# togheppi/pytorch-super-resolution-model-collection

Hardware: AMD Instinct MI355X
Metric: ESPCN x4 LR->HR images/sec (infer) (higher is better)
Workload: dtype f32 storage/accumulate; fp32-faithful products on the fp16 matrix cores: operands scaled by exact powers of two, split into two fp16 planes, 3 MFMAs per product (f16x3, ~3e-7 rms vs fp64, like fp32 MFMA); 1 GPU; c2: ESPCN x4 inference, 256x256 LR, batch 64 per GPU, fp32, random-init N(0,0.02); parallelism=replicas x1 (no collective)

## Files before the change

pytorch_super_resolution_model_collection_amd/csrc/conv_pair.hip:

```cpp
#include "srk_common.h"
#include "conv_problem.h"
#include "bf16_frag.h"
#include <type_traits>

namespace srk {

namespace {

constexpr int PR_TH = 8, PR_TW = 16, PR_HW = 18, PR_NPIX = 180, PR_NPIXP = 190;
constexpr int PR_XR = 14, PR_XC = 23, PR_XP = 24;
constexpr int PR_NSLOT = 3;
constexpr int PR_WL2 = 9 * 2 * 256;
constexpr int PR_HBUF = 8 * PR_NPIXP;
constexpr int PR_XBUF = 2 * PR_XR * PR_XP;
constexpr unsigned PR_SPIN_CAP = 1u << 18;
constexpr size_t PR_LDS = (size_t)PR_WL2 * 16 + (size_t)PR_NSLOT * PR_HBUF * 16 + (size_t)2 * PR_XBUF * 8 + 64;

__device__ unsigned g_pair_timeouts = 0;

typedef __attribute__((address_space(3))) unsigned pr_cnt_t;
typedef unsigned v4u_t __attribute__((ext_vector_type(4)));

struct PairParams {
  const float* x;
  const float* w1;
  const float* b1;
  const uint4* wq2;
  const float* w2_descale;
  const float* b2;
  float* y;
  const float* x_amax;
  float* y_amax;
  int N, H, W, OH, OW, tiles_x, img_tiles, ntiles;
  unsigned x_img_bytes, y_bytes;
};

__device__ __forceinline__ unsigned pr_peek(pr_cnt_t* p) {
  return (unsigned)__builtin_amdgcn_readfirstlane((int)__hip_atomic_load(p, __ATOMIC_RELAXED, __HIP_MEMORY_SCOPE_WORKGROUP));
}
__device__ __forceinline__ void pr_wait(pr_cnt_t* p, unsigned target, bool& dead) {
  if (!dead) {
    unsigned spins = 0;
    while ((int)(pr_peek(p) - target) < 0) {
      __builtin_amdgcn_s_sleep(1);
      if (++spins > PR_SPIN_CAP) {
        dead = true;
        break;
      }
    }
  }
  asm volatile("" ::: "memory");
}
__device__ __forceinline__ void pr_signal(pr_cnt_t* p) {
  asm volatile("" ::: "memory");
  if ((threadIdx.x & 63) == 0) __hip_atomic_fetch_add(p, 1u, __ATOMIC_RELAXED, __HIP_MEMORY_SCOPE_WORKGROUP);
  asm volatile("" ::: "memory");
}

__device__ __forceinline__ __amdgpu_buffer_rsrc_t pr_rsrc(const void* base, unsigned bytes) {
  const unsigned long long a = reinterpret_cast<unsigned long long>(base);
  const unsigned lo = __builtin_amdgcn_readfirstlane((unsigned)a), hi = __builtin_amdgcn_readfirstlane((unsigned)(a >> 32));
  void* p = reinterpret_cast<void*>(((unsigned long long)hi << 32) | lo);
  return __builtin_amdgcn_make_buffer_rsrc(p, (short)0, (int)__builtin_amdgcn_readfirstlane(bytes), 0x00020000);
}

__global__ __launch_bounds__(512, 1) void k_espcn_pair(PairParams B) {
  extern __shared__ __attribute__((aligned(16))) uint4 smem4[];
  uint4* wl2 = smem4;
  uint4* ring = smem4 + PR_WL2;
  uint2* xin_all = reinterpret_cast<uint2*>(ring + PR_NSLOT * PR_HBUF);
  pr_cnt_t* cnt = (pr_cnt_t*)(xin_all + 2 * PR_XBUF);
  const int tid = threadIdx.x, lane = tid & 63, wave = tid >> 6;
  const int grp = wave >> 2, gw = wave & 3, lt = tid & 255;
  const int j = lane & 15, kq = lane >> 4;
  uint2* xin = xin_all + grp * PR_XBUF;

  const float xmax = amax_read(B.x_amax);
  const int kx = amax_scale_exp(xmax);
  float wsum = 0.f, wmax = 0.f;
  {
    const float* wc = B.w1 + lane * 75;
    for (int i = 0; i < 75; ++i) {
      const float a = fabsf(wc[i]);
      wsum += a;
      wmax = fmaxf(wmax, a);
    }
  }
  const float bnd = wave_max(fabsf(B.b1[lane]) + wsum * xmax);
  const int kw1 = amax_scale_exp(wave_max(wmax));
  const int km = amax_scale_exp(bnd);
  const float sx1 = exp2i(kx), sw1 = exp2i(kw1), sxm = exp2i(km);
  const float dsc1 = exp2i(-kx) * exp2i(-kw1);
  const float dsc2 = exp2i(-km) * B.w2_descale[0];

  for (int e = tid; e < PR_WL2; e += 512) wl2[e] = B.wq2[e];
  if (tid < 8) cnt[tid] = 0u;

  const int nf1 = gw & 1, mh = gw >> 1;
  uint4 w1f[2][4][2];
#pragma unroll
  for (int cc = 0; cc < 2; ++cc) {
    const int co = cc * 32 + nf1 * 16 + j;
#pragma unroll
    for (int ks = 0; ks < 4; ++ks) {
      const int q = 4 * ks + kq, dy = q / 3, dx0 = 2 * (q - 3 * (q / 3));
      float f[8];
#pragma unroll
      for (int e = 0; e < 8; ++e) {
        const int dx = dx0 + (e >> 2), ci = e & 3;
        const bool on = q < 15 && ci < 3 && dx < 5;
        f[e] = on ? B.w1[((co * 3 + (on ? ci : 0)) * 5 + (on ? dy : 0)) * 5 + (on ? dx : 0)] : 0.f;
      }
      uint4 pl[2];
      split8h(f, sw1, pl);
      w1f[cc][ks][0] = pl[0];
      w1f[cc][ks][1] = pl[1];
    }
  }
  float b1v[2][4];
#pragma unroll
  for (int cc = 0; cc < 2; ++cc)
#pragma unroll
    for (int e = 0; e < 4; ++e) b1v[cc][e] = B.b1[cc * 32 + nf1 * 16 + 4 * kq + e];
  int koff[4], moff[6], mpix[6];
#pragma unroll
  for (int ks = 0; ks < 4; ++ks) {
    const int q = (4 * ks + kq) < 15 ? 4 * ks + kq : 14;
    koff[ks] = (q / 3) * PR_XP + 2 * (q - 3 * (q / 3));
  }
#pragma unroll
  for (int m = 0; m < 6; ++m) {
    const int p = (6 * mh + m) * 16 + j;
    mpix[m] = p;
    const int pc = p < PR_NPIX ? p : PR_NPIX - 1;
    moff[m] = (pc / PR_HW) * PR_XP + pc % PR_HW;
  }

  const int rh = gw >> 1, nf2 = gw & 1;
  const int pj = j < 4 ? 2 * j : (j < 12 ? 2 * j - 7 : 2 * j - 16);
  const int lane_b = (4 * rh) * PR_HW + pj + kq * PR_NPIXP;
  const int lane_a = kq * 32 + nf2 * 16 + j;
  float b2v[4];
#pragma unroll
  for (int e = 0; e < 4; ++e) b2v[e] = B.b2[nf2 * 16 + 4 * kq + e];

  const int nblk = gridDim.x, xcd = blockIdx.x & 7, bi = blockIdx.x >> 3;
  int first, count;
  {
    const int per_x = B.ntiles >> 3, rem_x = B.ntiles & 7;
    const int nb_x = (nblk + 7 - xcd) >> 3;
    const int tiles_x = per_x + (xcd < rem_x ? 1 : 0);
    const int start_x = xcd * per_x + (xcd < rem_x ? xcd : rem_x);
    first = start_x + bi;
    count = bi < tiles_x ? (tiles_x - bi + nb_x - 1) / nb_x : 0;
  }
  const int tstride = (nblk + 7 - xcd) >> 3;
  count = __builtin_amdgcn_readfirstlane(count);

  const __amdgpu_buffer_rsrc_t yr = pr_rsrc(B.y, B.y_bytes);
  const unsigned HW_ = (unsigned)(B.H * B.W);
  float xv[2][3];
  auto xload = [&](int i) {
    const bool valid = i < count;
    const int t = first + (valid ? i : 0) * tstride;
    const int n = t / B.img_tiles, rem = t - n * B.img_tiles;
    const int ty = rem / B.tiles_x, tx = rem - ty * B.tiles_x;
    const __amdgpu_buffer_rsrc_t xr = pr_rsrc(B.x + (size_t)n * 3 * HW_, B.x_img_bytes);
#pragma unroll
    for (int s = 0; s < 2; ++s) {
      const int q = lt + 256 * s, qy = q / PR_XC, qx = q - qy * PR_XC;
      const bool ok = valid && q < PR_XR * PR_XC;
      const unsigned o = ok ? 4u * (unsigned)((ty * PR_TH + qy) * B.W + tx * PR_TW + qx) : 0x80000000u;
#pragma unroll
      for (int c = 0; c < 3; ++c)
        xv[s][c] = __builtin_bit_cast(float, __builtin_amdgcn_raw_buffer_load_b32(xr, (int)(o + (ok ? 4u * c * HW_ : 0u)), 0, 0));
    }
  };
  bool dead = false;
  float amax = 0.f;
  xload(grp);
  __syncthreads();

  unsigned own = 0;
  for (int i = grp; i < count; i += 2, ++own) {
#pragma unroll
    for (int s = 0; s < 2; ++s) {
      const int q = lt + 256 * s;
      if (q < PR_XR * PR_XC) {
        const int qy = q / PR_XC, qx = q - qy * PR_XC;
        unsigned h01, m01, h2, m2;
        split2h(xv[s][0], xv[s][1], sx1, h01, m01);
        split2h(xv[s][2], 0.f, sx1, h2, m2);
        xin[qy * PR_XP + qx] = make_uint2(h01, h2);
        xin[PR_XR * PR_XP + qy * PR_XP + qx] = make_uint2(m01, m2);
      }
    }
    pr_signal(cnt + 6 + grp);
    xload(i + 2);
    pr_wait(cnt + 6 + grp, 4u * (own + 1), dead);

    f32x4 a1[2][6];
#pragma unroll
    for (int cc = 0; cc < 2; ++cc)
#pragma unroll
      for (int m = 0; m < 6; ++m) a1[cc][m] = (f32x4){0.f, 0.f, 0.f, 0.f};
#pragma unroll
    for (int ks = 0; ks < 4; ++ks) {
#pragma unroll
      for (int m = 0; m < 6; ++m) {
        const int pa = moff[m] + koff[ks];
        const uint2 h0 = xin[pa], h1 = xin[pa + 1];
        const uint2 l0 = xin[PR_XR * PR_XP + pa], l1 = xin[PR_XR * PR_XP + pa + 1];
        const uint4 xh = make_uint4(h0.x, h0.y, h1.x, h1.y), xm = make_uint4(l0.x, l0.y, l1.x, l1.y);
#pragma unroll
        for (int cc = 0; cc < 2; ++cc) {
          a1[cc][m] = mfma16h(w1f[cc][ks][0], xm, a1[cc][m]);
          a1[cc][m] = mfma16h(w1f[cc][ks][1], xh, a1[cc][m]);
          a1[cc][m] = mfma16h(w1f[cc][ks][0], xh, a1[cc][m]);
        }
      }
    }
#pragma unroll
    for (int cc = 0; cc < 2; ++cc) {
      const unsigned st = 2u * (unsigned)i + cc, slot = st % PR_NSLOT, use = st / PR_NSLOT;
      pr_wait(cnt + 3 + slot, 4u * use, dead);
      unsigned char* hb = reinterpret_cast<unsigned char*>(ring + slot * PR_HBUF);
      const int g8 = 2 * nf1 + (kq >> 1), half = kq & 1;
#pragma unroll
      for (int m = 0; m < 6; ++m) {
        if (mpix[m] < PR_NPIX) {
          float v[4];
#pragma unroll
          for (int e = 0; e < 4; ++e) v[e] = fmaxf(__builtin_fmaf(a1[cc][m][e], dsc1, b1v[cc][e]), 0.f);
          unsigned h01, m01, h23, m23;
          split2h(v[0], v[1], sxm, h01, m01);
          split2h(v[2], v[3], sxm, h23, m23);
          *reinterpret_cast<uint2*>(hb + ((size_t)(0 * 4 + g8) * PR_NPIXP + mpix[m]) * 16 + half * 8) = make_uint2(h01, h23);
          *reinterpret_cast<uint2*>(hb + ((size_t)(1 * 4 + g8) * PR_NPIXP + mpix[m]) * 16 + half * 8) = make_uint2(m01, m23);
        }
      }
      pr_signal(cnt + slot);
    }

    const int t = first + i * tstride;
    const int n = t / B.img_tiles, rem = t - n * B.img_tiles;
    const int ty = rem / B.tiles_x, tx = rem - ty * B.tiles_x;
    f32x4 acc[4];
#pragma unroll
    for (int r = 0; r < 4; ++r) acc[r] = (f32x4){0.f, 0.f, 0.f, 0.f};
#pragma unroll
    for (int cc = 0; cc < 2; ++cc) {
      const unsigned st = 2u * (unsigned)i + cc, slot = st % PR_NSLOT, use = st / PR_NSLOT;
      pr_wait(cnt + slot, 4u * (use + 1), dead);
      const uint4* hb = ring + slot * PR_HBUF + lane_b;
#pragma unroll
      for (int v = 0; v < 3; ++v) {
        uint4 fa[3][2];
#pragma unroll
        for (int u = 0; u < 3; ++u) {
          fa[u][0] = wl2[((u * 3 + v) * 2 + cc) * 256 + lane_a];
          fa[u][1] = wl2[((u * 3 + v) * 2 + cc) * 256 + 128 + lane_a];
        }
#pragma unroll
        for (int R = 0; R < 6; ++R) {
          const uint4 xh = hb[R * PR_HW + v], xm = hb[R * PR_HW + v + 4 * PR_NPIXP];
#pragma unroll
          for (int u = 0; u < 3; ++u) {
            const int r = R - u;
            if (r >= 0 && r < 4) {
              acc[r] = mfma16h(fa[u][0], xm, acc[r]);
              acc[r] = mfma16h(fa[u][1], xh, acc[r]);
              acc[r] = mfma16h(fa[u][0], xh, acc[r]);
            }
          }
        }
      }
      pr_signal(cnt + 3 + slot);
    }
    const int oc = tx * PR_TW + pj;
#pragma unroll
    for (int r = 0; r < 4; ++r) {
      const int orow = ty * PR_TH + 4 * rh + r;
      const bool ok = oc < B.OW && orow < B.OH;
      f32x4 v;
#pragma unroll
      for (int e = 0; e < 4; ++e) v[e] = fmaxf(__builtin_fmaf(acc[r][e], dsc2, b2v[e]), 0.f);
      if (ok) amax = fmaxf(amax, fmaxf(fmaxf(v[0], v[1]), fmaxf(v[2], v[3])));
      const unsigned o = ok ? 4u * (unsigned)(((n * B.OH + orow) * B.OW + oc) * 32 + nf2 * 16 + 4 * kq) : 0x80000000u;
      __builtin_amdgcn_raw_buffer_store_b128(__builtin_bit_cast(v4u_t, v), yr, (int)o, 0, 0);
    }
  }
  if (B.y_amax) amax_commit(B.y_amax, amax, blockIdx.x + wave, amax_peek(B.y_amax, blockIdx.x + wave));
  if (dead && lane == 0) atomicAdd(&g_pair_timeouts, 1u);
}

}

int espcn_pair_launch(int N, int H, int W, const float* x, const float* w1, const float* b1, const void* wp2,
                      const float* b2, float* y, const float* x_amax, float* y_amax, bool force, hipStream_t s) {
  if (N < 1 || H < 7 || W < 7 || !x_amax) return -1;
  const int OH = H - 6, OW = W - 6;
  const int tiles_y = (OH + PR_TH - 1) / PR_TH, tiles_x = (OW + PR_TW - 1) / PR_TW;
  const long ntiles = (long)N * tiles_y * tiles_x;
  const size_t x_img = (size_t)3 * H * W * 4, y_bytes = (size_t)N * OH * OW * 32 * 4;
  if (ntiles >= (1L << 29) || x_img >= (1ull << 31) || y_bytes >= (1ull << 31)) return -1;
  if (!force) {
    if ((double)OH * OW < 0.85 * (double)tiles_y * tiles_x * (PR_TH * PR_TW)) return -1;
    if (ntiles < 4L * kNumCU) return -1;
  }
  const size_t elems = (size_t)9 * 64 * 32;
  const char* prepared = reinterpret_cast<const char*>(wp2) + bf3_prepared_offset(elems);
  const char* fsec = prepared + f16_section_offset(64, 32, 9);
  PairParams B{};
  B.x = x; B.w1 = w1; B.b1 = b1; B.b2 = b2; B.y = y; B.x_amax = x_amax; B.y_amax = y_amax;
  B.wq2 = reinterpret_cast<const uint4*>(fsec);
  B.w2_descale = reinterpret_cast<const float*>(fsec + bf3_main_bytes(64, 32, 9));
  B.N = N; B.H = H; B.W = W; B.OH = OH; B.OW = OW; B.tiles_x = tiles_x; B.img_tiles = tiles_x * tiles_y;
  B.ntiles = (int)ntiles;
  B.x_img_bytes = (unsigned)x_img;
  B.y_bytes = (unsigned)y_bytes;
  int grid = kNumCU;
  if (grid > ntiles) grid = (int)ntiles;
  note_amax_written(y_amax != nullptr);
  static LdsLimit lim;
  lim.ensure(reinterpret_cast<const void*>(&k_espcn_pair), PR_LDS);
  note_kernel("k_espcn_pair");
  hipLaunchKernelGGL(k_espcn_pair, dim3(grid), dim3(512), PR_LDS, s, B);
  return check_launch("espcn_pair");
}

int pair_ring_timeouts(int reset) {
  unsigned v = 0;
  if (hipMemcpyFromSymbol(&v, HIP_SYMBOL(g_pair_timeouts), sizeof(v)) != hipSuccess) {
    (void)hipGetLastError();
    return -1;
  }
  if (reset && v) {
    const unsigned z = 0;
    (void)hipMemcpyToSymbol(HIP_SYMBOL(g_pair_timeouts), &z, sizeof(z));
  }
  return (int)v;
}

}

extern "C" int srk_espcn_pair_forward(int N, int H, int W, const float* x, const float* w1, const float* b1,
                                      const float* w2_packed_fwd, const float* b2, float* y, const float* x_amax,
                                      float* y_amax, int force, void* stream) {
  if (!x || !w1 || !b1 || !w2_packed_fwd || !b2 || !y || !x_amax) return SRK_ERR_UNSUPPORTED;
  if (((uintptr_t)x | (uintptr_t)y) % 16 != 0) return SRK_ERR_UNSUPPORTED;
  const int rc = srk::espcn_pair_launch(N, H, W, x, w1, b1, w2_packed_fwd, b2, y, x_amax, y_amax, force != 0,
                                        (hipStream_t)stream);
  return rc == -1 ? SRK_ERR_UNSUPPORTED : rc;
}
```

Before: 70360 images/s.

## Reuse conv1 halo rows across vertically adjacent tiles via keep buffers

Each block now gets a contiguous run of tiles ordered column-major (tx outer, ty inner). The two-row layer-1 halo at the bottom of one tile is kept in a new LDS keep ring and reused as the top halo of the next tile, so layer-1 recomputation drops from 10 rows to about 8 per tile. The work split changes from per-channel-half to per-pixel-half, with 5/4 fragment tiles alternating between waves. This adds extra counters and a more intricate producer/consumer protocol, which risks more sync stalls and deadlock timeouts. The contiguous assignment also loses the strided interleave across XCDs.

```diff
diff --git a/pytorch_super_resolution_model_collection_amd/csrc/conv_pair.hip b/pytorch_super_resolution_model_collection_amd/csrc/conv_pair.hip
--- a/pytorch_super_resolution_model_collection_amd/csrc/conv_pair.hip
+++ b/pytorch_super_resolution_model_collection_amd/csrc/conv_pair.hip
@@ -7,14 +7,19 @@
 
 namespace {
 
-constexpr int PR_TH = 8, PR_TW = 16, PR_HW = 18, PR_NPIX = 180, PR_NPIXP = 190;
+constexpr int PR_TH = 8, PR_TW = 16, PR_HW = 18;
+constexpr int PR_NSLOTPIX = 6 * PR_HW, PR_NPIXP = PR_NSLOTPIX + 2;
+constexpr int PR_NKEEP = 2 * PR_HW, PR_KP = PR_NKEEP + 2;
 constexpr int PR_XR = 14, PR_XC = 23, PR_XP = 24;
-constexpr int PR_NSLOT = 3;
+constexpr int PR_NSLOT = 3, PR_NKBUF = 3;
 constexpr int PR_WL2 = 9 * 2 * 256;
-constexpr int PR_HBUF = 8 * PR_NPIXP;
+constexpr int PR_HBUF = 4 * PR_NPIXP;
+constexpr int PR_KBUF = 2 * 4 * PR_KP;
+constexpr int PR_PLANE = PR_NSLOT * PR_HBUF + PR_NKBUF * PR_KBUF;
 constexpr int PR_XBUF = 2 * PR_XR * PR_XP;
 constexpr unsigned PR_SPIN_CAP = 1u << 18;
-constexpr size_t PR_LDS = (size_t)PR_WL2 * 16 + (size_t)PR_NSLOT * PR_HBUF * 16 + (size_t)2 * PR_XBUF * 8 + 64;
+constexpr size_t PR_LDS = (size_t)PR_WL2 * 16 + (size_t)2 * PR_PLANE * 16 + (size_t)2 * PR_XBUF * 8 + 64;
+static_assert(PR_LDS <= 160 * 1024, "k_espcn_pair: LDS");
 
 __device__ unsigned g_pair_timeouts = 0;
 
@@ -31,7 +36,7 @@
   float* y;
   const float* x_amax;
   float* y_amax;
-  int N, H, W, OH, OW, tiles_x, img_tiles, ntiles;
+  int N, H, W, OH, OW, tiles_y, img_tiles, ntiles;
   unsigned x_img_bytes, y_bytes;
 };
 
@@ -51,9 +56,9 @@
   }
   asm volatile("" ::: "memory");
 }
-__device__ __forceinline__ void pr_signal(pr_cnt_t* p) {
+__device__ __forceinline__ void pr_signal(pr_cnt_t* p, unsigned n = 1u) {
   asm volatile("" ::: "memory");
-  if ((threadIdx.x & 63) == 0) __hip_atomic_fetch_add(p, 1u, __ATOMIC_RELAXED, __HIP_MEMORY_SCOPE_WORKGROUP);
+  if ((threadIdx.x & 63) == 0) __hip_atomic_fetch_add(p, n, __ATOMIC_RELAXED, __HIP_MEMORY_SCOPE_WORKGROUP);
   asm volatile("" ::: "memory");
 }
 
@@ -68,7 +73,8 @@
   extern __shared__ __attribute__((aligned(16))) uint4 smem4[];
   uint4* wl2 = smem4;
   uint4* ring = smem4 + PR_WL2;
-  uint2* xin_all = reinterpret_cast<uint2*>(ring + PR_NSLOT * PR_HBUF);
+  uint4* keep = ring + PR_NSLOT * PR_HBUF;
+  uint2* xin_all = reinterpret_cast<uint2*>(ring + 2 * PR_PLANE);
   pr_cnt_t* cnt = (pr_cnt_t*)(xin_all + 2 * PR_XBUF);
   const int tid = threadIdx.x, lane = tid & 63, wave = tid >> 6;
   const int grp = wave >> 2, gw = wave & 3, lt = tid & 255;
@@ -94,13 +100,13 @@
   const float dsc2 = exp2i(-km) * B.w2_descale[0];
 
   for (int e = tid; e < PR_WL2; e += 512) wl2[e] = B.wq2[e];
-  if (tid < 8) cnt[tid] = 0u;
-
-  const int nf1 = gw & 1, mh = gw >> 1;
+  if (tid < 14) cnt[tid] = 0u;
+
+  const int c1 = gw >> 1, mh = gw & 1;
   uint4 w1f[2][4][2];
 #pragma unroll
-  for (int cc = 0; cc < 2; ++cc) {
-    const int co = cc * 32 + nf1 * 16 + j;
+  for (int nf = 0; nf < 2; ++nf) {
+    const int co = c1 * 32 + nf * 16 + j;
 #pragma unroll
     for (int ks = 0; ks < 4; ++ks) {
       const int q = 4 * ks + kq, dy = q / 3, dx0 = 2 * (q - 3 * (q / 3));
@@ -113,48 +119,47 @@
       }
       uint4 pl[2];
       split8h(f, sw1, pl);
-      w1f[cc][ks][0] = pl[0];
-      w1f[cc][ks][1] = pl[1];
-    }
-  }
-  float b1v[2][4];
-#pragma unroll
-  for (int cc = 0; cc < 2; ++cc)
-#pragma unroll
-    for (int e = 0; e < 4; ++e) b1v[cc][e] = B.b1[cc * 32 + nf1 * 16 + 4 * kq + e];
-  int koff[4], moff[6], mpix[6];
+      w1f[nf][ks][0] = pl[0];
+      w1f[nf][ks][1] = pl[1];
+    }
+  }
+  int koff[4], mpix[5], moff[5], tpix[2], toff[2];
 #pragma unroll
   for (int ks = 0; ks < 4; ++ks) {
     const int q = (4 * ks + kq) < 15 ? 4 * ks + kq : 14;
     koff[ks] = (q / 3) * PR_XP + 2 * (q - 3 * (q / 3));
   }
 #pragma unroll
-  for (int m = 0; m < 6; ++m) {
-    const int p = (6 * mh + m) * 16 + j;
-    mpix[m] = p;
-    const int pc = p < PR_NPIX ? p : PR_NPIX - 1;
-    moff[m] = (pc / PR_HW) * PR_XP + pc % PR_HW;
-  }
+  for (int m = 0; m < 5; ++m) {
+    mpix[m] = 16 * (m < 4 ? 4 * mh + m : 8) + j;
+    const int p = PR_NKEEP + mpix[m];
+    moff[m] = (p / PR_HW) * PR_XP + p % PR_HW;
+  }
+#pragma unroll
+  for (int m = 0; m < 2; ++m) {
+    tpix[m] = 16 * (2 * mh + m) + j;
+    const int p = tpix[m] < PR_NKEEP ? tpix[m] : PR_NKEEP - 1;
+    toff[m] = (p / PR_HW) * PR_XP + p % PR_HW;
+  }
+  const int wr_slot = (kq >> 1) * PR_NPIXP * 16 + (kq & 1) * 8, wr_keep = (c1 * 4 + (kq >> 1)) * PR_KP * 16 + (kq & 1) * 8;
 
   const int rh = gw >> 1, nf2 = gw & 1;
   const int pj = j < 4 ? 2 * j : (j < 12 ? 2 * j - 7 : 2 * j - 16);
-  const int lane_b = (4 * rh) * PR_HW + pj + kq * PR_NPIXP;
+  const int lane_b = (4 * rh - 2) * PR_HW + pj + kq * PR_NPIXP;
+  const int lane_k = pj + kq * PR_KP;
   const int lane_a = kq * 32 + nf2 * 16 + j;
   float b2v[4];
 #pragma unroll
   for (int e = 0; e < 4; ++e) b2v[e] = B.b2[nf2 * 16 + 4 * kq + e];
 
-  const int nblk = gridDim.x, xcd = blockIdx.x & 7, bi = blockIdx.x >> 3;
+  const int nblk = gridDim.x, xcd = blockIdx.x & 7;
   int first, count;
   {
-    const int per_x = B.ntiles >> 3, rem_x = B.ntiles & 7;
-    const int nb_x = (nblk + 7 - xcd) >> 3;
-    const int tiles_x = per_x + (xcd < rem_x ? 1 : 0);
-    const int start_x = xcd * per_x + (xcd < rem_x ? xcd : rem_x);
-    first = start_x + bi;
-    count = bi < tiles_x ? (tiles_x - bi + nb_x - 1) / nb_x : 0;
-  }
-  const int tstride = (nblk + 7 - xcd) >> 3;
+    const int lb = xcd * (nblk >> 3) + (xcd < (nblk & 7) ? xcd : (nblk & 7)) + (blockIdx.x >> 3);
+    const int per = B.ntiles / nblk, rem = B.ntiles - per * nblk;
+    first = lb * per + (lb < rem ? lb : rem);
+    count = per + (lb < rem ? 1 : 0);
+  }
   count = __builtin_amdgcn_readfirstlane(count);
 
   const __amdgpu_buffer_rsrc_t yr = pr_rsrc(B.y, B.y_bytes);
@@ -162,9 +167,9 @@
   float xv[2][3];
   auto xload = [&](int i) {
     const bool valid = i < count;
-    const int t = first + (valid ? i : 0) * tstride;
+    const int t = first + (valid ? i : 0);
     const int n = t / B.img_tiles, rem = t - n * B.img_tiles;
-    const int ty = rem / B.tiles_x, tx = rem - ty * B.tiles_x;
+    const int tx = rem / B.tiles_y, ty = rem - tx * B.tiles_y;
     const __amdgpu_buffer_rsrc_t xr = pr_rsrc(B.x + (size_t)n * 3 * HW_, B.x_img_bytes);
 #pragma unroll
     for (int s = 0; s < 2; ++s) {
@@ -174,6 +179,27 @@
 #pragma unroll
       for (int c = 0; c < 3; ++c)
         xv[s][c] = __builtin_bit_cast(float, __builtin_amdgcn_raw_buffer_load_b32(xr, (int)(o + (ok ? 4u * c * HW_ : 0u)), 0, 0));
+    }
+  };
+  auto l1_frags = [&](auto nm, const int* off, f32x4 (*a)[2]) {
+    constexpr int NM = decltype(nm)::value;
+#pragma unroll
+    for (int m = 0; m < NM; ++m) a[m][0] = a[m][1] = (f32x4){0.f, 0.f, 0.f, 0.f};
+#pragma unroll
+    for (int ks = 0; ks < 4; ++ks) {
+#pragma unroll
+      for (int m = 0; m < NM; ++m) {
+        const int pa = off[m] + koff[ks];
+        const uint2 h0 = xin[pa], h1 = xin[pa + 1];
+        const uint2 l0 = xin[PR_XR * PR_XP + pa], l1 = xin[PR_XR * PR_XP + pa + 1];
+        const uint4 xh = make_uint4(h0.x, h0.y, h1.x, h1.y), xm = make_uint4(l0.x, l0.y, l1.x, l1.y);
+#pragma unroll
+        for (int nf = 0; nf < 2; ++nf) {
+          a[m][nf] = mfma16h(w1f[nf][ks][0], xm, a[m][nf]);
+          a[m][nf] = mfma16h(w1f[nf][ks][1], xh, a[m][nf]);
+          a[m][nf] = mfma16h(w1f[nf][ks][0], xh, a[m][nf]);
+        }
+      }
     }
   };
   bool dead = false;
@@ -182,7 +208,18 @@
   __syncthreads();
 
   unsigned own = 0;
+  unsigned kseq = 0;
+  int typrev = 0;
   for (int i = grp; i < count; i += 2, ++own) {
+    const int t = first + i;
+    const int n = t / B.img_tiles, rem = t - n * B.img_tiles;
+    const int tx = rem / B.tiles_y, ty = rem - tx * B.tiles_y;
+    const bool fresh = i == 0 || ty == 0;
+    const bool hand = i + 1 < count && ty + 1 < B.tiles_y;
+    kseq = i == grp ? (grp == 0 ? 1u : 2u + (ty == 0 ? 1u : 0u))
+                    : kseq + 2u + (typrev + 1 == B.tiles_y ? 1u : 0u) + (ty == 0 ? 1u : 0u);
+    typrev = ty;
+    const unsigned kb = kseq % PR_NKBUF, ku = kseq / PR_NKBUF, tb = (kseq - 1u) % PR_NKBUF, tu = (kseq - 1u) / PR_NKBUF;
 #pragma unroll
     for (int s = 0; s < 2; ++s) {
       const int q = lt + 256 * s;
@@ -199,60 +236,69 @@
     xload(i + 2);
     pr_wait(cnt + 6 + grp, 4u * (own + 1), dead);
 
-    f32x4 a1[2][6];
-#pragma unroll
-    for (int cc = 0; cc < 2; ++cc)
-#pragma unroll
-      for (int m = 0; m < 6; ++m) a1[cc][m] = (f32x4){0.f, 0.f, 0.f, 0.f};
-#pragma unroll
-    for (int ks = 0; ks < 4; ++ks) {
-#pragma unroll
-      for (int m = 0; m < 6; ++m) {
-        const int pa = moff[m] + koff[ks];
-        const uint2 h0 = xin[pa], h1 = xin[pa + 1];
-        const uint2 l0 = xin[PR_XR * PR_XP + pa], l1 = xin[PR_XR * PR_XP + pa + 1];
-        const uint4 xh = make_uint4(h0.x, h0.y, h1.x, h1.y), xm = make_uint4(l0.x, l0.y, l1.x, l1.y);
-#pragma unroll
-        for (int cc = 0; cc < 2; ++cc) {
-          a1[cc][m] = mfma16h(w1f[cc][ks][0], xm, a1[cc][m]);
-          a1[cc][m] = mfma16h(w1f[cc][ks][1], xh, a1[cc][m]);
-          a1[cc][m] = mfma16h(w1f[cc][ks][0], xh, a1[cc][m]);
-        }
-      }
-    }
+    float b1v[2][4];
+#pragma unroll
+    for (int nf = 0; nf < 2; ++nf)
+#pragma unroll
+      for (int e = 0; e < 4; ++e) b1v[nf][e] = B.b1[c1 * 32 + nf * 16 + 4 * kq + e];
+    auto l1_store = [&](const f32x4 (&a)[2], unsigned char* base, int pix, int pitch) {
+#pragma unroll
+      for (int nf = 0; nf < 2; ++nf) {
+        float v[4];
+#pragma unroll
+        for (int e = 0; e < 4; ++e) v[e] = fmaxf(__builtin_fmaf(a[nf][e], dsc1, b1v[nf][e]), 0.f);
+        unsigned h01, m01, h23, m23;
+        split2h(v[0], v[1], sxm, h01, m01);
+        split2h(v[2], v[3], sxm, h23, m23);
+        *reinterpret_cast<uint2*>(base + ((2 * nf) * pitch + pix) * 16) = make_uint2(h01, h23);
+        *reinterpret_cast<uint2*>(base + (PR_PLANE + (2 * nf) * pitch + pix) * 16) = make_uint2(m01, m23);
+      }
+    };
+    auto l1_tile = [&](auto nm) {
+      constexpr int NM = decltype(nm)::value;
+      f32x4 a1[NM][2];
+      l1_frags(nm, moff, a1);
+      const unsigned st = 2u * (unsigned)i + c1, slot = st % PR_NSLOT, use = st / PR_NSLOT;
+      unsigned char* hb = reinterpret_cast<unsigned char*>(ring + slot * PR_HBUF) + wr_slot;
+      pr_wait(cnt + 3 + slot, 4u * use, dead);
+#pragma unroll
+      for (int m = 0; m < NM; ++m)
+        if (mpix[m] < PR_NSLOTPIX) l1_store(a1[m], hb, mpix[m], PR_NPIXP);
+      pr_signal(cnt + slot);
+      unsigned char* kp = reinterpret_cast<unsigned char*>(keep + kb * PR_KBUF) + wr_keep;
+      pr_wait(cnt + 11 + kb, 8u * ku, dead);
+#pragma unroll
+      for (int m = 2; m < NM; ++m)
+        if (mpix[m] >= PR_NSLOTPIX) l1_store(a1[m], kp, mpix[m] - PR_NSLOTPIX, PR_KP);
+      pr_signal(cnt + 8 + kb);
+    };
+    if (mh == (int)(own & 1))
+      l1_tile(std::integral_constant<int, 5>{});
+    else
+      l1_tile(std::integral_constant<int, 4>{});
+    if (fresh) {
+      f32x4 at[2][2];
+      l1_frags(std::integral_constant<int, 2>{}, toff, at);
+      unsigned char* kp = reinterpret_cast<unsigned char*>(keep + tb * PR_KBUF) + wr_keep;
+      pr_wait(cnt + 11 + tb, 8u * tu, dead);
+#pragma unroll
+      for (int m = 0; m < 2; ++m)
+        if (tpix[m] < PR_NKEEP) l1_store(at[m], kp, tpix[m], PR_KP);
+      pr_signal(cnt + 8 + tb);
+    }
+
+    f32x4 acc[4];
+#pragma unroll
+    for (int r = 0; r < 4; ++r) acc[r] = (f32x4){0.f, 0.f, 0.f, 0.f};
+    pr_wait(cnt + 8 + (rh == 0 ? tb : kb), 4u * ((rh == 0 ? tu : ku) + 1u), dead);
 #pragma unroll
     for (int cc = 0; cc < 2; ++cc) {
       const unsigned st = 2u * (unsigned)i + cc, slot = st % PR_NSLOT, use = st / PR_NSLOT;
-      pr_wait(cnt + 3 + slot, 4u * use, dead);
-      unsigned char* hb = reinterpret_cast<unsigned char*>(ring + slot * PR_HBUF);
-      const int g8 = 2 * nf1 + (kq >> 1), half = kq & 1;
-#pragma unroll
-      for (int m = 0; m < 6; ++m) {
-        if (mpix[m] < PR_NPIX) {
-          float v[4];
-#pragma unroll
-          for (int e = 0; e < 4; ++e) v[e] = fmaxf(__builtin_fmaf(a1[cc][m][e], dsc1, b1v[cc][e]), 0.f);
-          unsigned h01, m01, h23, m23;
-          split2h(v[0], v[1], sxm, h01, m01);
-          split2h(v[2], v[3], sxm, h23, m23);
-          *reinterpret_cast<uint2*>(hb + ((size_t)(0 * 4 + g8) * PR_NPIXP + mpix[m]) * 16 + half * 8) = make_uint2(h01, h23);
-          *reinterpret_cast<uint2*>(hb + ((size_t)(1 * 4 + g8) * PR_NPIXP + mpix[m]) * 16 + half * 8) = make_uint2(m01, m23);
-        }
-      }
-      pr_signal(cnt + slot);
-    }
-
-    const int t = first + i * tstride;
-    const int n = t / B.img_tiles, rem = t - n * B.img_tiles;
-    const int ty = rem / B.tiles_x, tx = rem - ty * B.tiles_x;
-    f32x4 acc[4];
-#pragma unroll
-    for (int r = 0; r < 4; ++r) acc[r] = (f32x4){0.f, 0.f, 0.f, 0.f};
-#pragma unroll
-    for (int cc = 0; cc < 2; ++cc) {
-      const unsigned st = 2u * (unsigned)i + cc, slot = st % PR_NSLOT, use = st / PR_NSLOT;
-      pr_wait(cnt + slot, 4u * (use + 1), dead);
+      pr_wait(cnt + slot, 2u * (use + 1), dead);
       const uint4* hb = ring + slot * PR_HBUF + lane_b;
+      const uint4* kr = keep + (rh == 0 ? tb : kb) * PR_KBUF + cc * 4 * PR_KP + lane_k - (rh == 0 ? 0 : 4 * PR_HW);
+      const uint4* pa = rh == 0 ? kr : hb;
+      const uint4* pc = rh == 0 ? hb : kr;
 #pragma unroll
       for (int v = 0; v < 3; ++v) {
         uint4 fa[3][2];
@@ -263,7 +309,8 @@
         }
 #pragma unroll
         for (int R = 0; R < 6; ++R) {
-          const uint4 xh = hb[R * PR_HW + v], xm = hb[R * PR_HW + v + 4 * PR_NPIXP];
+          const uint4* px = R < 2 ? pa : (R < 4 ? hb : pc);
+          const uint4 xh = px[R * PR_HW + v], xm = px[R * PR_HW + v + PR_PLANE];
 #pragma unroll
           for (int u = 0; u < 3; ++u) {
             const int r = R - u;
@@ -277,6 +324,8 @@
       }
       pr_signal(cnt + 3 + slot);
     }
+    pr_signal(cnt + 11 + tb, fresh ? 2u : 1u);
+    pr_signal(cnt + 11 + kb, hand ? 1u : 2u);
     const int oc = tx * PR_TW + pj;
 #pragma unroll
     for (int r = 0; r < 4; ++r) {
@@ -315,7 +364,7 @@
   B.x = x; B.w1 = w1; B.b1 = b1; B.b2 = b2; B.y = y; B.x_amax = x_amax; B.y_amax = y_amax;
   B.wq2 = reinterpret_cast<const uint4*>(fsec);
   B.w2_descale = reinterpret_cast<const float*>(fsec + bf3_main_bytes(64, 32, 9));
-  B.N = N; B.H = H; B.W = W; B.OH = OH; B.OW = OW; B.tiles_x = tiles_x; B.img_tiles = tiles_x * tiles_y;
+  B.N = N; B.H = H; B.W = W; B.OH = OH; B.OW = OW; B.tiles_y = tiles_y; B.img_tiles = tiles_x * tiles_y;
   B.ntiles = (int)ntiles;
   B.x_img_bytes = (unsigned)x_img;
   B.y_bytes = (unsigned)y_bytes;
```

Measured after the change: 72570 images/s, median of 6. 1.03x the previous value.
